# glaretechnologies/substrata

Measured on AMD Instinct MI355X. Metric: physics steps/sec at fixed dt, 100k bodies, higher is better.
Workload: dtype f32; 1 GPU; BASELINE config 3: 100000 mixed box/sphere/capsule bodies, 100x100x10 lattice spacing 1.5 m, seed 3, ground quad 2000 m, dt 1/60, Jolt default settings (10 velocity / 2 position iterations), sleeping enabled; bodies_per_gpu=100000, tiles=1, active_bodies_end=99193, contact_constraints_start=296641, contact_constraints_end=299690, contact_points_end=362045, colours_end=21, contact_constraints_after_settle=293058, dropped_pairs_or_manifolds=0

## Files before the change

substrata_amd/csrc/sgp_k_broadphase.hip:

```cpp
#include "sgp_dev_all.h"

__global__ void __launch_bounds__(TPB) k_step_begin(DV d, StepParams sp, uint32_t nb, int reset_scratch, uint32_t bounds_blocks, int ev_reset)
{
	const uint32_t tid = blockIdx.x * TPB + threadIdx.x, stride = gridDim.x * TPB;
	if (ev_reset && tid < sizeof(EventCounters) / 4) ((uint32_t*)d.evc)[tid] = 0u;
	if (tid == 0) {
		const uint32_t par = reset_scratch ? (d.sp->parity ^ 1u) : d.sp->parity;
		*d.sp = sp;
		d.sp->parity = par;
		*d.veh_epoch = *d.veh_epoch + 1u;
	}
	uint32_t* c = (uint32_t*)d.ctr;
	for (uint32_t i = tid; i < sizeof(StepCounters) / 4; i += stride) c[i] = 0;
	const uint32_t used = min(*d.grid_cells_used, d.table_size) + 4u;
	for (uint32_t i = tid; i < used; i += stride) { d.cell_count[i] = 0; d.cell_fill[i] = 0; }
	for (uint32_t sl = tid; sl < (used - 4u) / 64u; sl += stride) d.tile_slot[d.tile_of_slot[sl]] = BP_TILE_NONE;
	if (reset_scratch) {
		const uint32_t n = min(nb, d.cap_bodies);
		for (uint32_t i = tid; i < n; i += stride) { d.colour_mask[i] = 0ull; d.claim[0][i] = ~0ull; d.claim[1][i] = ~0ull; }
	}
	if (blockIdx.x >= bounds_blocks) return;
	float mnx = 3.0e38f, mny = 3.0e38f, mnz = 3.0e38f, mxx = -3.0e38f, mxy = -3.0e38f, mxz = -3.0e38f;
	const uint32_t n_slots = sp.n_slots;
	for (uint32_t i = tid; i < n_slots; i += bounds_blocks * TPB) {
		const uint32_t f = d.flags[i];
		if ((f & BF_ALIVE) && !(f & BF_LARGE)) {
			const float4 mn = d.aabb_min[i], mx = d.aabb_max[i];
			const float cx = (mn.x + mx.x) * 0.5f, cy = (mn.y + mx.y) * 0.5f, cz = (mn.z + mx.z) * 0.5f;
			mnx = fminf(mnx, cx); mny = fminf(mny, cy); mnz = fminf(mnz, cz); mxx = fmaxf(mxx, cx); mxy = fmaxf(mxy, cy); mxz = fmaxf(mxz, cz);
		}
	}
	for (int off = 32; off > 0; off >>= 1) {
		mnx = fminf(mnx, __shfl_down(mnx, off, 64)); mny = fminf(mny, __shfl_down(mny, off, 64)); mnz = fminf(mnz, __shfl_down(mnz, off, 64));
		mxx = fmaxf(mxx, __shfl_down(mxx, off, 64)); mxy = fmaxf(mxy, __shfl_down(mxy, off, 64)); mxz = fmaxf(mxz, __shfl_down(mxz, off, 64));
	}
	__shared__ float red[6][TPB / 64];
	if ((threadIdx.x & 63) == 0) { const int wv = threadIdx.x >> 6; red[0][wv] = mnx; red[1][wv] = mny; red[2][wv] = mnz; red[3][wv] = mxx; red[4][wv] = mxy; red[5][wv] = mxz; }
	__syncthreads();
	if (threadIdx.x < 6) {
		float v = red[threadIdx.x][0];
		for (int k = 1; k < TPB / 64; ++k) v = threadIdx.x < 3 ? fminf(v, red[threadIdx.x][k]) : fmaxf(v, red[threadIdx.x][k]);
		int* dst = d.bounds_acc + threadIdx.x;
		if (threadIdx.x < 3) { if (v < 2.9e38f) atomicMin(dst, float_to_ordered(v)); }
		else { if (v > -2.9e38f) atomicMax(dst, float_to_ordered(v)); }
	}
}

__global__ void k_set_params(DV d, StepParams sp) { if (threadIdx.x == 0 && blockIdx.x == 0) *d.sp = sp; }

__global__ void __launch_bounds__(TPB) k_step_end(DV d, StepCounters* host_mapped, EventWindow* host_events) { step_end_block(d, host_mapped, host_events); }

__global__ void __launch_bounds__(TPB) k_fill_u64(uint64_t* p, uint64_t v, size_t n)
{
	for (size_t i = (size_t)blockIdx.x * TPB + threadIdx.x; i < n; i += (size_t)gridDim.x * TPB) p[i] = v;
}


SGP_DEV BpGrid bp_grid_from_bounds(const DV& d)
{
	BpGrid g;
	g.min_x = d.bounds_acc[0]; g.min_y = d.bounds_acc[1]; g.min_z = d.bounds_acc[2]; g.max_x = d.bounds_acc[3]; g.max_y = d.bounds_acc[4]; g.max_z = d.bounds_acc[5];
	g.ox = g.oy = g.oz = 0.0f; g.nx = g.ny = g.nz = 1;
	float cell = d.sp->cell_size;
	if (g.min_x <= g.max_x) {
		const float x0 = ordered_to_float(g.min_x), y0 = ordered_to_float(g.min_y), z0 = ordered_to_float(g.min_z);
		const float x1 = ordered_to_float(g.max_x), y1 = ordered_to_float(g.max_y), z1 = ordered_to_float(g.max_z);
		for (int it = 0; it < 64; ++it) {
			const float inv = 1.0f / cell;
			const float fx = floorf((x1 - x0) * inv) + 1.0f, fy = floorf((y1 - y0) * inv) + 1.0f, fz = floorf((z1 - z0) * inv) + 1.0f;
			const float tx = floorf((fx + 3.0f) * 0.25f), ty = floorf((fy + 3.0f) * 0.25f), tz = floorf((fz + 3.0f) * 0.25f);
			if (tx * ty * tz <= (float)d.tile_table_size && fx < 2.0e9f && fy < 2.0e9f && fz < 2.0e9f) { g.nx = (int)fx; g.ny = (int)fy; g.nz = (int)fz; break; }
			cell = cell * 1.5f;
			g.nx = g.ny = g.nz = 1;
		}
		g.ox = x0; g.oy = y0; g.oz = z0;
	}
	g.cell = cell; g.inv_cell = 1.0f / cell;
	g.n_cells = 1u;
	g.tnx = (g.nx + 3) >> 2; g.tny = (g.ny + 3) >> 2; g.tnz = (g.nz + 3) >> 2;
	return g;
}

SGP_DEV uint32_t grid_cell(const DV& d, const BpGrid& g, int x, int y, int z)
{
	const uint32_t slot = d.tile_slot[((uint32_t)(z >> 2) * (uint32_t)g.tny + (uint32_t)(y >> 2)) * (uint32_t)g.tnx + (uint32_t)(x >> 2)];
	return slot >= BP_TILE_PENDING ? BP_TILE_NONE : slot * 64u + (uint32_t)((((z & 3) << 2) | (y & 3)) << 2 | (x & 3));
}

__global__ void __launch_bounds__(TPB) k_bp_cell(DV d)
{
	__shared__ BpGrid sg;
	if (threadIdx.x == 0) {
		sg = bp_grid_from_bounds(d);
		if (blockIdx.x == 0) *d.grid = sg;
	}
	__syncthreads();
	const uint32_t i = blockIdx.x * TPB + threadIdx.x;
	const bool in_range = i < d.sp->n_slots;
	const uint32_t f = in_range ? d.flags[i] : 0u;
	uint32_t h = 0xFFFFFFFFu, tile = 0, local = 0;
	bool binned = false;
	const BpGrid& g = sg;
	if ((f & BF_ALIVE) && !(f & BF_LARGE)) {
		const float4 mn = d.aabb_min[i], mx = d.aabb_max[i];
		int cx = (int)floorf(((mn.x + mx.x) * 0.5f - g.ox) * g.inv_cell);
		int cy = (int)floorf(((mn.y + mx.y) * 0.5f - g.oy) * g.inv_cell);
		int cz = (int)floorf(((mn.z + mx.z) * 0.5f - g.oz) * g.inv_cell);
		cx = min(max(cx, 0), g.nx - 1); cy = min(max(cy, 0), g.ny - 1); cz = min(max(cz, 0), g.nz - 1);
		tile = ((uint32_t)(cz >> 2) * (uint32_t)g.tny + (uint32_t)(cy >> 2)) * (uint32_t)g.tnx + (uint32_t)(cx >> 2);
		local = (uint32_t)((((cz & 3) << 2) | (cy & 3)) << 2 | (cx & 3));
		binned = true;
	}
	const int lane = (int)(threadIdx.x & 63u);
	int leader = lane;
	for (int k = 0; k < 64; ++k) {
		const uint32_t tk = (uint32_t)__shfl((int)tile, k, 64);
		const int bk = __shfl((int)binned, k, 64);
		if (bk && binned && tk == tile && k < leader) leader = k;
	}
	uint32_t sl = BP_TILE_NONE;
	const bool leads = binned && leader == lane;
	uint32_t* const entry = &d.tile_slot[leads ? tile : 0u];
	if (leads) sl = __hip_atomic_load(entry, __ATOMIC_RELAXED, __HIP_MEMORY_SCOPE_AGENT);
	bool won = false;
	if (leads && sl >= BP_TILE_PENDING) {
		const uint32_t old = atomicCAS(entry, BP_TILE_NONE, BP_TILE_PENDING);
		if (old == BP_TILE_NONE) won = true; else sl = old;
	}
	{
		const unsigned long long wm = __ballot(won);
		if (wm) {
			uint32_t base = 0;
			const int first = __ffsll((long long)wm) - 1;
			if (lane == first) base = atomicAdd(&d.ctr->n_tiles_used, (uint32_t)__popcll(wm));
			base = (uint32_t)__shfl((int)base, first, 64);
			if (won) {
				sl = base + (uint32_t)__popcll(wm & ((1ull << lane) - 1ull));
				d.tile_of_slot[sl] = tile;
				__hip_atomic_store(entry, sl, __ATOMIC_RELAXED, __HIP_MEMORY_SCOPE_AGENT);
			}
		}
	}
	if (leads) for (int tries = 0; tries < (1 << 24) && sl >= BP_TILE_PENDING; ++tries) sl = __hip_atomic_load(entry, __ATOMIC_RELAXED, __HIP_MEMORY_SCOPE_AGENT);
	const uint32_t slot = (uint32_t)__shfl((int)sl, leader, 64);
	if (binned) {
		if (slot >= BP_TILE_PENDING) { h = 0xFFFFFFFFu; if (lane == leader) atomicAdd(&d.ctr->pairs_dropped, 1u); }
		else { h = slot * 64u + local; atomicAdd(&d.cell_count[h], 1u); }
	}
	if (in_range) d.cell_hash[i] = h;
}

__global__ void __launch_bounds__(TPB) k_scan_blocks(const uint32_t* in, uint32_t* out, uint32_t* block_sums, uint32_t n_cap, const uint32_t* n_live)
{
	__shared__ uint32_t wave_sums[TPB / 64];
	const uint32_t n = min(n_cap, *n_live * 64u + 1u);
	for (uint32_t blk = blockIdx.x; blk * (TPB * 4u) < n; blk += gridDim.x) {
	__syncthreads();
	const uint32_t base = (blk * TPB + threadIdx.x) * 4;
	uint32_t v[4];
#pragma unroll
	for (int k = 0; k < 4; ++k) v[k] = (base + k < n) ? in[base + k] : 0u;
	const uint32_t tsum = v[0] + v[1] + v[2] + v[3];
	uint32_t x = tsum;
	const int lane = threadIdx.x & 63;
#pragma unroll
	for (int off = 1; off < 64; off <<= 1) { const uint32_t y = __shfl_up(x, off, 64); if (lane >= off) x += y; }
	const int wave = threadIdx.x >> 6;
	if (lane == 63) wave_sums[wave] = x;
	__syncthreads();
	uint32_t wbase = 0;
	for (int k = 0; k < wave; ++k) wbase += wave_sums[k];
	uint32_t excl = wbase + x - tsum;
#pragma unroll
	for (int k = 0; k < 4; ++k) { if (base + k < n) out[base + k] = excl; excl += v[k]; }
	if (threadIdx.x == TPB - 1) block_sums[blk] = wbase + x;
	}
}

__global__ void __launch_bounds__(1024) k_scan_sums(uint32_t* block_sums, uint32_t nb_cap, uint32_t n_cap, const uint32_t* n_live, uint32_t* cells_used_out)
{
	const uint32_t nb = min(nb_cap, (min(n_cap, *n_live * 64u + 1u) + TPB * 4u - 1u) / (TPB * 4u));
	if (threadIdx.x == 0) *cells_used_out = min(n_cap, *n_live * 64u);
	__shared__ uint32_t wave_sums[16];
	__shared__ uint32_t carry;
	if (threadIdx.x == 0) carry = 0;
	__syncthreads();
	for (uint32_t start = 0; start < nb; start += 1024) {
		const uint32_t i = start + threadIdx.x;
		const uint32_t v = i < nb ? block_sums[i] : 0u;
		uint32_t x = v;
		const int lane = threadIdx.x & 63, wave = threadIdx.x >> 6;
#pragma unroll
		for (int off = 1; off < 64; off <<= 1) { const uint32_t y = __shfl_up(x, off, 64); if (lane >= off) x += y; }
		if (lane == 63) wave_sums[wave] = x;
		__syncthreads();
		uint32_t wbase = carry;
		for (int k = 0; k < wave; ++k) wbase += wave_sums[k];
		if (i < nb) block_sums[i] = wbase + x - v;
		__syncthreads();
		if (threadIdx.x == 1023) carry = wbase + x;
		__syncthreads();
	}
}

__global__ void __launch_bounds__(TPB) k_scan_add(uint32_t* out, const uint32_t* block_sums, uint32_t n_cap, const uint32_t* n_live)
{
	const uint32_t n = min(n_cap, *n_live * 64u + 1u);
	for (uint32_t blk = blockIdx.x; blk * (TPB * 4u) < n; blk += gridDim.x) {
		const uint32_t base = (blk * TPB + threadIdx.x) * 4;
		const uint32_t add = block_sums[blk];
#pragma unroll
		for (int k = 0; k < 4; ++k) if (base + k < n) out[base + k] += add;
	}
}

SGP_DEV void bp_scatter_one(const DV& d, uint32_t i)
{
	if (i < 6u) d.bounds_acc[i] = i < 3u ? 0x7FFFFFFF : (int)0x80000000;
	if (i >= d.sp->n_slots) return;
	const uint32_t h = d.cell_hash[i];
	if (h == 0xFFFFFFFFu) return;
	const uint32_t slot = d.cell_start[h] + atomicAdd(&d.cell_fill[h], 1u);
	const float4 mn = d.aabb_min[i], mx = d.aabb_max[i];
	d.sorted_min[slot] = make_float4(mn.x, mn.y, mn.z, __uint_as_float(d.flags[i]));
	d.sorted_max[slot] = make_float4(mx.x, mx.y, mx.z, __uint_as_float(i));
}
__global__ void __launch_bounds__(TPB) k_bp_scatter(DV d) { bp_scatter_one(d, blockIdx.x * TPB + threadIdx.x); }

SGP_DEV bool rec_pair_passes(float spec, float4 mni, float4 mxi, float4 mnj, float4 mxj)
{
	const uint32_t fi = __float_as_uint(mni.w), fj = __float_as_uint(mnj.w);
	if (f_motion(fi) != SGP_MOTION_DYNAMIC && f_motion(fj) != SGP_MOTION_DYNAMIC) return false;
	if (!layers_collide(f_layer(fi), f_layer(fj))) return false;
	if (mni.x - spec > mxj.x || mnj.x - spec > mxi.x) return false;
	if (mni.y - spec > mxj.y || mnj.y - spec > mxi.y) return false;
	if (mni.z - spec > mxj.z || mnj.z - spec > mxi.z) return false;
	return true;
}
SGP_DEV void push_pair(const DV& d, uint32_t i, uint32_t j)
{
	const uint32_t k = wave_alloc(&d.ctr->n_pairs);
	if (k < d.cap_pairs) d.pairs[k] = make_uint2(i < j ? i : j, i < j ? j : i);
	else atomicAdd(&d.ctr->pairs_dropped, 1u);
}

template <int PCAP> SGP_DEV void stage_pair(const DV& d, uint2* spairs, uint8_t* scls, uint32_t* lcount, uint32_t i, uint32_t j, uint32_t fi, uint32_t fj);

#define BP_TILE 4
#define BP_H 2
#define BP_HALO (BP_TILE + 2 * BP_H)
#define BP_HALO_CELLS (BP_HALO * BP_HALO * BP_HALO)
#define BP_INNER_CELLS (BP_TILE * BP_TILE * BP_TILE)
#ifndef BP_LDS_CAP_SMALL
#define BP_LDS_CAP_SMALL 768
#endif
#ifndef BP_PAIR_CAP_SMALL
#define BP_PAIR_CAP_SMALL 1024
#endif
#define BP_LDS_CAP_LARGE 1536
#define BP_PAIR_CAP_LARGE 2048
#ifndef BP_SPLIT
#define BP_SPLIT 4
#endif

SGP_DEV uint32_t pair_class(uint32_t fa, uint32_t fb) { const uint32_t ta = f_shape(fa), tb = f_shape(fb); return (ta < tb ? ta : tb) * 8u + (ta < tb ? tb : ta); }
template <int PCAP> SGP_DEV void stage_pair(const DV& d, uint2* spairs, uint8_t* scls, uint32_t* lcount, uint32_t i, uint32_t j, uint32_t fi, uint32_t fj)
{
	const uint32_t k = atomicAdd(lcount, 1u);
	if (k < (uint32_t)PCAP) { spairs[k] = make_uint2(i < j ? i : j, i < j ? j : i); scls[k] = (uint8_t)pair_class(fi, fj); }
	else push_pair(d, i, j);
}
template <int PCAP> SGP_DEV void flush_pairs(const DV& d, const uint2* spairs, const uint8_t* scls, uint32_t lcount, uint32_t* gbase, uint32_t* bins)
{
	const uint32_t n_out = min(lcount, (uint32_t)PCAP);
	if (threadIdx.x < 64) bins[threadIdx.x] = 0;
	if (threadIdx.x == 0 && n_out) *gbase = atomicAdd(&d.ctr->n_pairs, n_out);
	__syncthreads();
	uint32_t rank[PCAP / TPB];
#pragma unroll
	for (int r = 0; r < PCAP / TPB; ++r) { const uint32_t k = threadIdx.x + (uint32_t)r * TPB; rank[r] = k < n_out ? atomicAdd(&bins[scls[k]], 1u) : 0u; }
	__syncthreads();
	if (threadIdx.x < 64) {
		const uint32_t v = bins[threadIdx.x];
		uint32_t x = v;
#pragma unroll
		for (int off = 1; off < 64; off <<= 1) { const uint32_t y = __shfl_up(x, off, 64); if ((int)threadIdx.x >= off) x += y; }
		bins[threadIdx.x] = x - v;
	}
	__syncthreads();
#pragma unroll
	for (int r = 0; r < PCAP / TPB; ++r) {
		const uint32_t k = threadIdx.x + (uint32_t)r * TPB;
		if (k < n_out) {
			const uint32_t at = *gbase + bins[scls[k]] + rank[r];
			if (at < d.cap_pairs) d.pairs[at] = spairs[k];
			else atomicAdd(&d.ctr->pairs_dropped, 1u);
		}
	}
}

SGP_DEV uint32_t block_scan_512(uint32_t* a, int n, uint32_t* wave_tot)
{
	const int t = threadIdx.x;
	const uint32_t v0 = (2 * t < n) ? a[2 * t] : 0u, v1 = (2 * t + 1 < n) ? a[2 * t + 1] : 0u;
	uint32_t x = v0 + v1;
	const int lane = t & 63, wave = t >> 6;
	for (int off = 1; off < 64; off <<= 1) { const uint32_t y = __shfl_up(x, off, 64); if (lane >= off) x += y; }
	if (lane == 63) wave_tot[wave] = x;
	__syncthreads();
	uint32_t base = 0, total = 0;
	for (int k = 0; k < TPB / 64; ++k) { if (k < wave) base += wave_tot[k]; total += wave_tot[k]; }
	const uint32_t excl = base + x - (v0 + v1);
	__syncthreads();
	if (2 * t < n) a[2 * t] = excl;
	if (2 * t + 1 < n) a[2 * t + 1] = excl + v0;
	__syncthreads();
	return total;
}

template <int BP_LDS_CAP, int BP_PAIR_CAP> __global__ void __launch_bounds__(TPB) k_bp_pairs(DV d)
{
	__shared__ float4 smin[BP_LDS_CAP];
	__shared__ float4 smax[BP_LDS_CAP];
	__shared__ uint32_t cstart[BP_HALO_CELLS + 1];
	__shared__ uint32_t gstart[BP_HALO_CELLS];
	__shared__ uint32_t istart[BP_INNER_CELLS + 1];
	__shared__ uint32_t wave_tot[TPB / 64];
	__shared__ uint2 spairs[BP_PAIR_CAP];
	__shared__ uint8_t scls[BP_PAIR_CAP];
	__shared__ uint32_t pbins[64];
	__shared__ uint32_t lcount, gbase;
	__shared__ uint32_t nslot[27];
	const BpGrid g = *d.grid;
	const uint32_t n_tiles = d.ctr->n_tiles_used;
	const float spec = d.st.speculative_contact_distance;
	const float reach = d.sp->bp_rmax + spec;
	if (threadIdx.x == 0) lcount = 0;
	for (uint32_t slot = blockIdx.x; slot < n_tiles; slot += gridDim.x) {
		const uint32_t tile = d.tile_of_slot[slot];
		const int tx = (int)(tile % (uint32_t)g.tnx), ty = (int)((tile / (uint32_t)g.tnx) % (uint32_t)g.tny), tz = (int)(tile / ((uint32_t)g.tnx * (uint32_t)g.tny));
		const int x0 = tx * BP_TILE - BP_H, y0 = ty * BP_TILE - BP_H, z0 = tz * BP_TILE - BP_H;
		__syncthreads();
		if (threadIdx.x < BP_INNER_CELLS) {
			const uint32_t lin = slot * 64u + threadIdx.x;
			istart[threadIdx.x] = d.cell_start[lin + 1] - d.cell_start[lin];
		} else if (threadIdx.x < BP_INNER_CELLS + 27) {
			const int k = (int)threadIdx.x - BP_INNER_CELLS;
			const int nx_ = tx + k % 3 - 1, ny_ = ty + (k / 3) % 3 - 1, nz_ = tz + k / 9 - 1;
			nslot[k] = (nx_ >= 0 && nx_ < g.tnx && ny_ >= 0 && ny_ < g.tny && nz_ >= 0 && nz_ < g.tnz) ? d.tile_slot[((uint32_t)nz_ * (uint32_t)g.tny + (uint32_t)ny_) * (uint32_t)g.tnx + (uint32_t)nx_] : BP_TILE_NONE;
		}
		__syncthreads();
		const uint32_t n_inner = block_scan_512(istart, BP_INNER_CELLS, wave_tot);
		if (threadIdx.x == 0) istart[BP_INNER_CELLS] = n_inner;
		if (n_inner == 0) continue;
		for (int c = threadIdx.x; c < BP_HALO_CELLS; c += TPB) {
			const int hx = c % BP_HALO, hy = (c / BP_HALO) % BP_HALO, hz = c / (BP_HALO * BP_HALO);
			const int x = x0 + hx, y = y0 + hy, z = z0 + hz;
			uint32_t b = 0, cnt = 0;
			if (x >= 0 && x < g.nx && y >= 0 && y < g.ny && z >= 0 && z < g.nz) {
				const uint32_t ns = nslot[(((z >> 2) - tz + 1) * 3 + ((y >> 2) - ty + 1)) * 3 + ((x >> 2) - tx + 1)];
				if (ns < BP_TILE_PENDING) { const uint32_t lin = ns * 64u + (uint32_t)((((z & 3) << 2) | (y & 3)) << 2 | (x & 3)); b = d.cell_start[lin]; cnt = d.cell_start[lin + 1] - b; }
			}
			gstart[c] = b;
			cstart[c] = cnt;
		}
		__syncthreads();
		const uint32_t total = block_scan_512(cstart, BP_HALO_CELLS, wave_tot);
		if (threadIdx.x == 0) cstart[BP_HALO_CELLS] = total;
		__syncthreads();
		const bool in_lds = total <= (uint32_t)BP_LDS_CAP;
		if (threadIdx.x == 0 && total > (uint32_t)BP_LDS_CAP_SMALL) d.ctr->bp_dense = 1u;
		if (in_lds) {
			for (uint32_t q = threadIdx.x; q < total; q += TPB) {
				int lo = 0, hi = BP_HALO_CELLS - 1;
				while (lo < hi) { const int mid = (lo + hi + 1) >> 1; if (cstart[mid] <= q) lo = mid; else hi = mid - 1; }
				const uint32_t src = gstart[lo] + (q - cstart[lo]);
				smin[q] = d.sorted_min[src]; smax[q] = d.sorted_max[src];
			}
		}
		__syncthreads();
		for (uint32_t tt = threadIdx.x; tt < n_inner * BP_SPLIT; tt += TPB) {
			const uint32_t t = tt / BP_SPLIT;
			const int sub = (int)(tt % BP_SPLIT);
			int lo = 0, hi = BP_INNER_CELLS - 1;
			while (lo < hi) { const int mid = (lo + hi + 1) >> 1; if (istart[mid] <= t) lo = mid; else hi = mid - 1; }
			const int ic = lo;
			const uint32_t k = t - istart[ic];
			const int ix = ic % BP_TILE, iy = (ic / BP_TILE) % BP_TILE, iz = ic / (BP_TILE * BP_TILE);
			const int hc = ((iz + BP_H) * BP_HALO + (iy + BP_H)) * BP_HALO + (ix + BP_H);
			const float4 mni = in_lds ? smin[cstart[hc] + k] : d.sorted_min[gstart[hc] + k];
			const float4 mxi = in_lds ? smax[cstart[hc] + k] : d.sorted_max[gstart[hc] + k];
			const uint32_t fi = __float_as_uint(mni.w), i = __float_as_uint(mxi.w);
			if (!f_active_for_pairs(fi)) continue;
			int xl = (int)floorf((mni.x - reach - g.ox) * g.inv_cell) - x0, xh = (int)floorf((mxi.x + reach - g.ox) * g.inv_cell) - x0;
			int yl = (int)floorf((mni.y - reach - g.oy) * g.inv_cell) - y0, yh = (int)floorf((mxi.y + reach - g.oy) * g.inv_cell) - y0;
			int zl = (int)floorf((mni.z - reach - g.oz) * g.inv_cell) - z0, zh = (int)floorf((mxi.z + reach - g.oz) * g.inv_cell) - z0;
			xl = min(max(xl, 0), ix + BP_H); xh = max(min(xh, BP_HALO - 1), ix + BP_H);
			yl = min(max(yl, 0), iy + BP_H); yh = max(min(yh, BP_HALO - 1), iy + BP_H);
			zl = min(max(zl, 0), iz + BP_H); zh = max(min(zh, BP_HALO - 1), iz + BP_H);
			const int ny_rows = yh - yl + 1, n_rows = (zh - zl + 1) * ny_rows;
			for (int row = sub; row < n_rows; row += BP_SPLIT) {
				const int hz = zl + row / ny_rows, hy = yl + row % ny_rows;
				const int rb = (hz * BP_HALO + hy) * BP_HALO;
				if (in_lds) {
					const uint32_t q0 = cstart[rb + xl], q1 = cstart[rb + xh + 1];
					for (uint32_t q = q0; q < q1; ++q) {
						const float4 mnj = smin[q], mxj = smax[q];
						const uint32_t j = __float_as_uint(mxj.w);
						if (j == i) continue;
						if (f_active_for_pairs(__float_as_uint(mnj.w)) && j < i) continue;
						if (rec_pair_passes(spec, mni, mxi, mnj, mxj)) stage_pair<BP_PAIR_CAP>(d, spairs, scls, &lcount, i, j, fi, __float_as_uint(mnj.w));
					}
				} else {
					for (int c = xl; c <= xh; ++c) {
						const uint32_t gb = gstart[rb + c], gn = cstart[rb + c + 1] - cstart[rb + c];
						for (uint32_t q = 0; q < gn; ++q) {
							const float4 mnj = d.sorted_min[gb + q], mxj = d.sorted_max[gb + q];
							const uint32_t j = __float_as_uint(mxj.w);
							if (j == i) continue;
							if (f_active_for_pairs(__float_as_uint(mnj.w)) && j < i) continue;
							if (rec_pair_passes(spec, mni, mxi, mnj, mxj)) stage_pair<BP_PAIR_CAP>(d, spairs, scls, &lcount, i, j, fi, __float_as_uint(mnj.w));
						}
					}
				}
			}
		}
		__syncthreads();
		if (lcount > BP_PAIR_CAP / 2) {
			flush_pairs<BP_PAIR_CAP>(d, spairs, scls, lcount, &gbase, pbins);
			__syncthreads();
			if (threadIdx.x == 0) lcount = 0;
		}
	}
	__syncthreads();
	flush_pairs<BP_PAIR_CAP>(d, spairs, scls, lcount, &gbase, pbins);
}
__global__ void __launch_bounds__(TPB) k_gather_aabbs(DV d, const uint32_t* ids, uint32_t n, float4* out)
{
	const uint32_t k = blockIdx.x * TPB + threadIdx.x;
	if (k >= n) return;
	out[2 * (size_t)k] = d.aabb_min[ids[k]]; out[2 * (size_t)k + 1] = d.aabb_max[ids[k]];
}
SGP_DEV void bp_large_one(const DV& d, uint32_t j)
{
	const uint32_t fj = j < d.sp->n_slots ? d.flags[j] : 0u;
	const bool live_j = (fj & BF_ALIVE) && !(fj & BF_ALIAS);
	float4 mnj = make_float4(0.0f, 0.0f, 0.0f, 0.0f), mxj = mnj;
	if (live_j) { mnj = d.aabb_min[j]; mxj = d.aabb_max[j]; }
	for (uint32_t l = 0; l < d.sp->n_large; ++l) {
		const uint32_t i = d.large_ids[l];
		bool pair = false;
		if (live_j && i != j) {
			const uint32_t fi = d.flags[i];
			pair = (fi & BF_ALIVE) && !((fj & BF_LARGE) && j < i)
			       && (f_active_for_pairs(fi) || f_active_for_pairs(fj)) && pair_passes(d, fj, mnj, mxj, i);
		}
		const uint32_t k = block_alloc(&d.ctr->n_pairs, pair);
		if (pair) { if (k < d.cap_pairs) d.pairs[k] = make_uint2(i < j ? i : j, i < j ? j : i); else atomicAdd(&d.ctr->pairs_dropped, 1u); }
	}
	if (live_j && f_active_for_pairs(fj)) {
		const float s = d.st.speculative_contact_distance;
		large_grid_query(d, V3(mnj.x - s, mnj.y - s, mnj.z - s), V3(mxj.x + s, mxj.y + s, mxj.z + s), [&](uint32_t i) {
			if (i == j || !pair_passes(d, fj, mnj, mxj, i)) return;
			if ((fj & BF_LARGE) && j < i) return;
			const uint32_t k = wave_alloc(&d.ctr->n_pairs);
			if (k < d.cap_pairs) d.pairs[k] = make_uint2(i < j ? i : j, i < j ? j : i); else atomicAdd(&d.ctr->pairs_dropped, 1u);
		});
	}
}
__global__ void __launch_bounds__(TPB) k_bp_large(DV d) { bp_large_one(d, blockIdx.x * TPB + threadIdx.x); }
__global__ void __launch_bounds__(TPB) k_bp_scatter_large(DV d) { const uint32_t i = blockIdx.x * TPB + threadIdx.x; bp_scatter_one(d, i); bp_large_one(d, i); }

void launch_step_begin(const DV& d, const StepParams& sp, uint32_t nb, bool reset_step_scratch, bool ev_reset, hipStream_t s)
{
	const uint32_t work = std::max(d.table_size + 4, reset_step_scratch ? nb : 0u);
	uint32_t blocks = (work + TPB * 4 - 1) / (TPB * 4);
	if (blocks < 1) blocks = 1; if (blocks > 1024) blocks = 1024;
	hipLaunchKernelGGL(k_step_begin, dim3(blocks), dim3(TPB), 0, s, d, sp, nb, reset_step_scratch ? 1 : 0, std::min(blocks, std::min(blocks_for(nb), 128u)), ev_reset ? 1 : 0);
}
void launch_set_params(const DV& d, const StepParams& sp, hipStream_t s) { hipLaunchKernelGGL(k_set_params, dim3(1), dim3(64), 0, s, d, sp); }
void launch_step_end(const DV& d, StepCounters* host_mapped, EventWindow* host_events, hipStream_t s) { hipLaunchKernelGGL(k_step_end, dim3(1), dim3(TPB), 0, s, d, host_mapped, host_events); }
void launch_fill_u64(uint64_t* p, uint64_t v, size_t n, hipStream_t s)
{
	size_t blocks = (n + TPB * 8 - 1) / (TPB * 8);
	if (blocks < 1) blocks = 1; if (blocks > 2048) blocks = 2048;
	hipLaunchKernelGGL(k_fill_u64, dim3((uint32_t)blocks), dim3(TPB), 0, s, p, v, n);
}
void launch_bp_bounds(const DV&, uint32_t, hipStream_t) {}
void launch_bp_cell(const DV& d, uint32_t nb, hipStream_t s) { hipLaunchKernelGGL(k_bp_cell, dim3(blocks_for(nb)), dim3(TPB), 0, s, d); }
void launch_bp_scan(const DV& d, hipStream_t s)
{
	const uint32_t n = d.table_size + 1;
	const uint32_t nb = (n + 1023) / 1024;
	const uint32_t* n_tiles = &d.ctr->n_tiles_used;
	const uint32_t grid = std::min(nb, 1024u);
	hipLaunchKernelGGL(k_scan_blocks, dim3(grid), dim3(TPB), 0, s, d.cell_count, d.cell_start, d.scan_block_sums, n, n_tiles);
	hipLaunchKernelGGL(k_scan_sums, dim3(1), dim3(1024), 0, s, d.scan_block_sums, nb, n, n_tiles, d.grid_cells_used);
	hipLaunchKernelGGL(k_scan_add, dim3(grid), dim3(TPB), 0, s, d.cell_start, d.scan_block_sums, n, n_tiles);
}
void launch_bp_scatter(const DV& d, uint32_t nb, hipStream_t s) { hipLaunchKernelGGL(k_bp_scatter, dim3(blocks_for(nb)), dim3(TPB), 0, s, d); }
void launch_bp_pairs(const DV& d, int small_lds, hipStream_t s)
{
	if (small_lds) hipLaunchKernelGGL((k_bp_pairs<BP_LDS_CAP_SMALL, BP_PAIR_CAP_SMALL>), dim3(4096), dim3(TPB), 0, s, d);
	else hipLaunchKernelGGL((k_bp_pairs<BP_LDS_CAP_LARGE, BP_PAIR_CAP_LARGE>), dim3(4096), dim3(TPB), 0, s, d);
}
void launch_bp_large(const DV& d, uint32_t nb, hipStream_t s) { hipLaunchKernelGGL(k_bp_large, dim3(blocks_for(nb)), dim3(TPB), 0, s, d); }
void launch_bp_scatter_large(const DV& d, uint32_t nb, hipStream_t s) { hipLaunchKernelGGL(k_bp_scatter_large, dim3(blocks_for(nb)), dim3(TPB), 0, s, d); }
void launch_gather_aabbs(const DV& d, const uint32_t* ids, uint32_t n, float4* out, hipStream_t s) { if (n) hipLaunchKernelGGL(k_gather_aabbs, dim3(blocks_for(n)), dim3(TPB), 0, s, d, ids, n, out); }
```

Baseline: 598.5 steps/s.

## Restructure broadphase tile setup: prefetch tile heads, fuse scans, branchless pair test

The pair kernel now prefetches the next tile's header (tile id and inner cell_start bounds) while processing the current one. It derives inner cell offsets directly from the sorted cell_start instead of running a block scan, and has each thread own two adjacent halo cells so that a single wave scan replaces the second block scan. It also swaps the binary-search copy into LDS for per-thread direct copies and adds a byte lookup table mapping item to inner cell. The inner candidate loop software-prefetches the next LDS entry and uses a branchless combined test, aiming to cut barriers, binary searches and divergence at the cost of more register pressure and more complex code.

```diff
diff --git a/substrata_amd/csrc/sgp_k_broadphase.hip b/substrata_amd/csrc/sgp_k_broadphase.hip
--- a/substrata_amd/csrc/sgp_k_broadphase.hip
+++ b/substrata_amd/csrc/sgp_k_broadphase.hip
@@ -236,6 +236,17 @@
 	if (mni.y - spec > mxj.y || mnj.y - spec > mxi.y) return false;
 	if (mni.z - spec > mxj.z || mnj.z - spec > mxi.z) return false;
 	return true;
+}
+SGP_DEV bool bp_candidate_passes(float spec, uint32_t i, float4 mni, float4 mxi, float4 mnj, float4 mxj)
+{
+	const uint32_t fi = __float_as_uint(mni.w), fj = __float_as_uint(mnj.w), j = __float_as_uint(mxj.w);
+	const uint32_t li = f_layer(fi), lj = f_layer(fj);
+	const bool mine = (j != i) & !(((fj & (BF_ALIVE | BF_ACTIVE)) == (BF_ALIVE | BF_ACTIVE)) & (f_motion(fj) != SGP_MOTION_STATIC) & (j < i));
+	const bool moves = (f_motion(fi) == SGP_MOTION_DYNAMIC) | (f_motion(fj) == SGP_MOTION_DYNAMIC);
+	const bool layers = ((li == SGP_LAYER_NON_MOVING) & (lj == SGP_LAYER_MOVING))
+	                    | ((li == SGP_LAYER_MOVING) & (lj != SGP_LAYER_NON_MOVING_NON_COLLIDABLE) & (lj != SGP_LAYER_MOVING_NON_COLLIDABLE));
+	const bool apart = (mni.x - spec > mxj.x) | (mnj.x - spec > mxi.x) | (mni.y - spec > mxj.y) | (mnj.y - spec > mxi.y) | (mni.z - spec > mxj.z) | (mnj.z - spec > mxi.z);
+	return mine & moves & layers & !apart;
 }
 SGP_DEV void push_pair(const DV& d, uint32_t i, uint32_t j)
 {
@@ -274,7 +285,8 @@
 {
 	const uint32_t n_out = min(lcount, (uint32_t)PCAP);
 	if (threadIdx.x < 64) bins[threadIdx.x] = 0;
-	if (threadIdx.x == 0 && n_out) *gbase = atomicAdd(&d.ctr->n_pairs, n_out);
+	uint32_t gb = 0;
+	if (threadIdx.x == 0 && n_out) gb = atomicAdd(&d.ctr->n_pairs, n_out);
 	__syncthreads();
 	uint32_t rank[PCAP / TPB];
 #pragma unroll
@@ -287,6 +299,7 @@
 		for (int off = 1; off < 64; off <<= 1) { const uint32_t y = __shfl_up(x, off, 64); if ((int)threadIdx.x >= off) x += y; }
 		bins[threadIdx.x] = x - v;
 	}
+	if (threadIdx.x == 0) *gbase = gb;
 	__syncthreads();
 #pragma unroll
 	for (int r = 0; r < PCAP / TPB; ++r) {
@@ -299,23 +312,15 @@
 	}
 }
 
-SGP_DEV uint32_t block_scan_512(uint32_t* a, int n, uint32_t* wave_tot)
-{
-	const int t = threadIdx.x;
-	const uint32_t v0 = (2 * t < n) ? a[2 * t] : 0u, v1 = (2 * t + 1 < n) ? a[2 * t + 1] : 0u;
-	uint32_t x = v0 + v1;
-	const int lane = t & 63, wave = t >> 6;
-	for (int off = 1; off < 64; off <<= 1) { const uint32_t y = __shfl_up(x, off, 64); if (lane >= off) x += y; }
-	if (lane == 63) wave_tot[wave] = x;
-	__syncthreads();
-	uint32_t base = 0, total = 0;
-	for (int k = 0; k < TPB / 64; ++k) { if (k < wave) base += wave_tot[k]; total += wave_tot[k]; }
-	const uint32_t excl = base + x - (v0 + v1);
-	__syncthreads();
-	if (2 * t < n) a[2 * t] = excl;
-	if (2 * t + 1 < n) a[2 * t + 1] = excl + v0;
-	__syncthreads();
-	return total;
+struct BpTileHead { uint32_t tile, cs0, cs64, mine; };
+SGP_DEV BpTileHead bp_tile_head(const DV& d, uint32_t slot)
+{
+	const uint32_t lin = min(slot, d.table_size / 64u - 1u) * 64u;
+	BpTileHead h;
+	h.tile = d.tile_of_slot[lin / 64u];
+	h.cs0 = d.cell_start[lin]; h.cs64 = d.cell_start[lin + 64u];
+	h.mine = d.cell_start[lin + min(threadIdx.x, 64u)];
+	return h;
 }
 
 template <int BP_LDS_CAP, int BP_PAIR_CAP> __global__ void __launch_bounds__(TPB) k_bp_pairs(DV d)
@@ -324,72 +329,103 @@
 	__shared__ float4 smax[BP_LDS_CAP];
 	__shared__ uint32_t cstart[BP_HALO_CELLS + 1];
 	__shared__ uint32_t gstart[BP_HALO_CELLS];
-	__shared__ uint32_t istart[BP_INNER_CELLS + 1];
+	__shared__ uint32_t ibase[BP_INNER_CELLS + 1];
 	__shared__ uint32_t wave_tot[TPB / 64];
 	__shared__ uint2 spairs[BP_PAIR_CAP];
 	__shared__ uint8_t scls[BP_PAIR_CAP];
 	__shared__ uint32_t pbins[64];
 	__shared__ uint32_t lcount, gbase;
 	__shared__ uint32_t nslot[27];
+	constexpr uint32_t BP_BCELL = 64u * sizeof(uint32_t);
+	uint8_t* const bcell = (uint8_t*)pbins;
+	static_assert(BP_HALO_CELLS == 2 * TPB && BP_HALO % 2 == 0 && BP_H % 2 == 0 && BP_TILE == 4, "a thread owns two halo cells that are neighbours in x inside one tile");
+	BpTileHead next = bp_tile_head(d, blockIdx.x);
 	const BpGrid g = *d.grid;
 	const uint32_t n_tiles = d.ctr->n_tiles_used;
 	const float spec = d.st.speculative_contact_distance;
 	const float reach = d.sp->bp_rmax + spec;
 	if (threadIdx.x == 0) lcount = 0;
 	for (uint32_t slot = blockIdx.x; slot < n_tiles; slot += gridDim.x) {
-		const uint32_t tile = d.tile_of_slot[slot];
+		const BpTileHead h = next;
+		next = bp_tile_head(d, slot + gridDim.x);
+		const uint32_t tile = h.tile;
 		const int tx = (int)(tile % (uint32_t)g.tnx), ty = (int)((tile / (uint32_t)g.tnx) % (uint32_t)g.tny), tz = (int)(tile / ((uint32_t)g.tnx * (uint32_t)g.tny));
 		const int x0 = tx * BP_TILE - BP_H, y0 = ty * BP_TILE - BP_H, z0 = tz * BP_TILE - BP_H;
-		__syncthreads();
-		if (threadIdx.x < BP_INNER_CELLS) {
-			const uint32_t lin = slot * 64u + threadIdx.x;
-			istart[threadIdx.x] = d.cell_start[lin + 1] - d.cell_start[lin];
-		} else if (threadIdx.x < BP_INNER_CELLS + 27) {
-			const int k = (int)threadIdx.x - BP_INNER_CELLS;
+		const uint32_t n_inner = h.cs64 - h.cs0;
+		__syncthreads();
+		if (n_inner == 0) continue;
+		if (threadIdx.x <= BP_INNER_CELLS) ibase[threadIdx.x] = h.mine;
+		else if (threadIdx.x >= 128 && threadIdx.x < 128 + 27) {
+			const int k = (int)threadIdx.x - 128;
 			const int nx_ = tx + k % 3 - 1, ny_ = ty + (k / 3) % 3 - 1, nz_ = tz + k / 9 - 1;
 			nslot[k] = (nx_ >= 0 && nx_ < g.tnx && ny_ >= 0 && ny_ < g.tny && nz_ >= 0 && nz_ < g.tnz) ? d.tile_slot[((uint32_t)nz_ * (uint32_t)g.tny + (uint32_t)ny_) * (uint32_t)g.tnx + (uint32_t)nx_] : BP_TILE_NONE;
 		}
 		__syncthreads();
-		const uint32_t n_inner = block_scan_512(istart, BP_INNER_CELLS, wave_tot);
-		if (threadIdx.x == 0) istart[BP_INNER_CELLS] = n_inner;
-		if (n_inner == 0) continue;
-		for (int c = threadIdx.x; c < BP_HALO_CELLS; c += TPB) {
+		if (threadIdx.x < BP_INNER_CELLS) {
+			const uint32_t t1 = min(ibase[threadIdx.x + 1] - h.cs0, BP_BCELL);
+			for (uint32_t t = ibase[threadIdx.x] - h.cs0; t < t1; ++t) bcell[t] = (uint8_t)threadIdx.x;
+		}
+		uint32_t b = 0, cnt0 = 0, cnt1 = 0;
+		{
+			const int c = 2 * (int)threadIdx.x;
 			const int hx = c % BP_HALO, hy = (c / BP_HALO) % BP_HALO, hz = c / (BP_HALO * BP_HALO);
 			const int x = x0 + hx, y = y0 + hy, z = z0 + hz;
-			uint32_t b = 0, cnt = 0;
 			if (x >= 0 && x < g.nx && y >= 0 && y < g.ny && z >= 0 && z < g.nz) {
-				const uint32_t ns = nslot[(((z >> 2) - tz + 1) * 3 + ((y >> 2) - ty + 1)) * 3 + ((x >> 2) - tx + 1)];
-				if (ns < BP_TILE_PENDING) { const uint32_t lin = ns * 64u + (uint32_t)((((z & 3) << 2) | (y & 3)) << 2 | (x & 3)); b = d.cell_start[lin]; cnt = d.cell_start[lin + 1] - b; }
+				uint32_t e0 = 0, e1 = 0;
+				if (hx >= BP_H && hx < BP_H + BP_TILE && hy >= BP_H && hy < BP_H + BP_TILE && hz >= BP_H && hz < BP_H + BP_TILE) {
+					const int ic = ((hz - BP_H) * BP_TILE + (hy - BP_H)) * BP_TILE + (hx - BP_H);
+					b = ibase[ic]; e0 = ibase[ic + 1]; e1 = ibase[ic + 2];
+				} else {
+					const uint32_t ns = nslot[(((z >> 2) - tz + 1) * 3 + ((y >> 2) - ty + 1)) * 3 + ((x >> 2) - tx + 1)];
+					if (ns < BP_TILE_PENDING) {
+						const uint32_t lin = ns * 64u + (uint32_t)((((z & 3) << 2) | (y & 3)) << 2 | (x & 3));
+						b = d.cell_start[lin]; e0 = d.cell_start[lin + 1]; e1 = d.cell_start[lin + 2];
+					}
+				}
+				cnt0 = e0 - b;
+				if (x + 1 < g.nx) cnt1 = e1 - e0;
 			}
-			gstart[c] = b;
-			cstart[c] = cnt;
-		}
-		__syncthreads();
-		const uint32_t total = block_scan_512(cstart, BP_HALO_CELLS, wave_tot);
+		}
+		uint32_t excl, total = 0;
+		{
+			uint32_t x = cnt0 + cnt1;
+			const int lane = threadIdx.x & 63, wave = threadIdx.x >> 6;
+			for (int off = 1; off < 64; off <<= 1) { const uint32_t y = __shfl_up(x, off, 64); if (lane >= off) x += y; }
+			if (lane == 63) wave_tot[wave] = x;
+			__syncthreads();
+			uint32_t base = 0;
+			for (int k = 0; k < TPB / 64; ++k) { if (k < wave) base += wave_tot[k]; total += wave_tot[k]; }
+			excl = base + x - (cnt0 + cnt1);
+		}
+		cstart[2 * threadIdx.x] = excl; cstart[2 * threadIdx.x + 1] = excl + cnt0;
+		gstart[2 * threadIdx.x] = b; gstart[2 * threadIdx.x + 1] = b + cnt0;
 		if (threadIdx.x == 0) cstart[BP_HALO_CELLS] = total;
-		__syncthreads();
 		const bool in_lds = total <= (uint32_t)BP_LDS_CAP;
 		if (threadIdx.x == 0 && total > (uint32_t)BP_LDS_CAP_SMALL) d.ctr->bp_dense = 1u;
 		if (in_lds) {
-			for (uint32_t q = threadIdx.x; q < total; q += TPB) {
-				int lo = 0, hi = BP_HALO_CELLS - 1;
-				while (lo < hi) { const int mid = (lo + hi + 1) >> 1; if (cstart[mid] <= q) lo = mid; else hi = mid - 1; }
-				const uint32_t src = gstart[lo] + (q - cstart[lo]);
-				smin[q] = d.sorted_min[src]; smax[q] = d.sorted_max[src];
+			const uint32_t n = cnt0 + cnt1;
+			for (uint32_t k = 0; k < n; k += 2) {
+				const uint32_t k1 = min(k + 1, n - 1);
+				const float4 a0 = d.sorted_min[b + k], a1 = d.sorted_max[b + k], c0 = d.sorted_min[b + k1], c1 = d.sorted_max[b + k1];
+				smin[excl + k] = a0; smax[excl + k] = a1; smin[excl + k1] = c0; smax[excl + k1] = c1;
 			}
 		}
 		__syncthreads();
 		for (uint32_t tt = threadIdx.x; tt < n_inner * BP_SPLIT; tt += TPB) {
 			const uint32_t t = tt / BP_SPLIT;
 			const int sub = (int)(tt % BP_SPLIT);
-			int lo = 0, hi = BP_INNER_CELLS - 1;
-			while (lo < hi) { const int mid = (lo + hi + 1) >> 1; if (istart[mid] <= t) lo = mid; else hi = mid - 1; }
-			const int ic = lo;
-			const uint32_t k = t - istart[ic];
+			int ic;
+			if (t < BP_BCELL) ic = bcell[t];
+			else {
+				int lo = 0, hi = BP_INNER_CELLS - 1;
+				while (lo < hi) { const int mid = (lo + hi + 1) >> 1; if (ibase[mid] - h.cs0 <= t) lo = mid; else hi = mid - 1; }
+				ic = lo;
+			}
+			const uint32_t k = t - (ibase[ic] - h.cs0);
 			const int ix = ic % BP_TILE, iy = (ic / BP_TILE) % BP_TILE, iz = ic / (BP_TILE * BP_TILE);
 			const int hc = ((iz + BP_H) * BP_HALO + (iy + BP_H)) * BP_HALO + (ix + BP_H);
-			const float4 mni = in_lds ? smin[cstart[hc] + k] : d.sorted_min[gstart[hc] + k];
-			const float4 mxi = in_lds ? smax[cstart[hc] + k] : d.sorted_max[gstart[hc] + k];
+			const float4 mni = in_lds ? smin[cstart[hc] + k] : d.sorted_min[h.cs0 + t];
+			const float4 mxi = in_lds ? smax[cstart[hc] + k] : d.sorted_max[h.cs0 + t];
 			const uint32_t fi = __float_as_uint(mni.w), i = __float_as_uint(mxi.w);
 			if (!f_active_for_pairs(fi)) continue;
 			int xl = (int)floorf((mni.x - reach - g.ox) * g.inv_cell) - x0, xh = (int)floorf((mxi.x + reach - g.ox) * g.inv_cell) - x0;
@@ -404,12 +440,15 @@
 				const int rb = (hz * BP_HALO + hy) * BP_HALO;
 				if (in_lds) {
 					const uint32_t q0 = cstart[rb + xl], q1 = cstart[rb + xh + 1];
-					for (uint32_t q = q0; q < q1; ++q) {
-						const float4 mnj = smin[q], mxj = smax[q];
-						const uint32_t j = __float_as_uint(mxj.w);
-						if (j == i) continue;
-						if (f_active_for_pairs(__float_as_uint(mnj.w)) && j < i) continue;
-						if (rec_pair_passes(spec, mni, mxi, mnj, mxj)) stage_pair<BP_PAIR_CAP>(d, spairs, scls, &lcount, i, j, fi, __float_as_uint(mnj.w));
+					if (q0 < q1) {
+						float4 mnj = smin[q0], mxj = smax[q0];
+						for (uint32_t q = q0; ; ) {
+							const uint32_t qn = min(q + 1, q1 - 1);
+							const float4 mnn = smin[qn], mxn = smax[qn];
+							if (bp_candidate_passes(spec, i, mni, mxi, mnj, mxj)) stage_pair<BP_PAIR_CAP>(d, spairs, scls, &lcount, i, __float_as_uint(mxj.w), fi, __float_as_uint(mnj.w));
+							if (++q >= q1) break;
+							mnj = mnn; mxj = mxn;
+						}
 					}
 				} else {
 					for (int c = xl; c <= xh; ++c) {
```

New measurement: 602.1 steps/s (median of 6 runs). About the same (+0.6%).
